# swyoon/Diffusion-by-MaxEntIRL

Hardware: AMD Instinct MI355X
Metric: images/sec (CIFAR-10 DDPM T=10 generation) (higher is better)
Workload: dtype bf16; 1 GPU; CIFAR-10 DDPM U-Net (35.7M params) VARSampler T=10 generation, 256 images/GPU/step, 3x32x32 (BASELINE configs[1]); noise drawn inside the step; global_batch=256, T=10, parallelism=dp1 (independent trajectories, no collective)

## Files before the change

### diffusion-by-maxentirl_amd/csrc/conv_common.h

```cpp
#pragma once
#include "common.h"

struct ConvArgs {
    const bf16* in0;
    const bf16* in1;
    const bf16* w;
    const float* bias;
    const float* addvec;
    const bf16* residual;
    const bf16* mask_src;
    void* out;
    int N, IH, IW, C0, C1, OH, OW, Cout;
    int ksize, stride, pad, ups, act, addvec_ld, in_mode, out_mode;
    int P, pre_act;
    int TWl, THl, SUBS;
    int HH, HWd;
    int PT, CT, CB, KST;
    int tile_px;
    int lds_buf;
    float mask_slope;
    int stagger;
    int RP, SP;
    float* gn_stats;
    bf16* gn_out;
    const float* gn_gamma;
    const float* gn_beta;
    float gn_eps;
    int gn_flags;
    int res_is_mask;
    int xcd_order;
};

__device__ __forceinline__ int dxmi_xcd_logical(int b, int G, int on) {
    if (!on) return b;
    const int x = b & 7, k = b >> 3;
    const int q = G >> 3, r = G & 7;
    return x * q + (x < r ? x : r) + k;
}

__device__ __forceinline__ float dxmi_row16_sum(float t) {
#define DXMI_DPP_ADD(ctrl) t += __builtin_bit_cast(float, __builtin_amdgcn_update_dpp(0, __builtin_bit_cast(int, t), ctrl, 0xf, 0xf, false))
    DXMI_DPP_ADD(0xB1);
    DXMI_DPP_ADD(0x4E);
    DXMI_DPP_ADD(0x141);
    DXMI_DPP_ADD(0x140);
#undef DXMI_DPP_ADD
    return t;
}

__device__ __forceinline__ void dxmi_stats4(const bf16x4& o, float (&st)[4]) {
    const bf16x2 lo = {o[0], o[1]}, hi = {o[2], o[3]};
    const bf16x2 one = {(bf16)1.f, (bf16)1.f};
    st[0] = __builtin_amdgcn_fdot2_f32_bf16(lo, one, st[0], false);
    st[1] = __builtin_amdgcn_fdot2_f32_bf16(lo, lo, st[1], false);
    st[2] = __builtin_amdgcn_fdot2_f32_bf16(hi, one, st[2], false);
    st[3] = __builtin_amdgcn_fdot2_f32_bf16(hi, hi, st[3], false);
}

__device__ __forceinline__ bool conv_block_to_tile(const ConvArgs& p, int bid, int& pt, int& cot) {
    const int xcd = bid & 7;
    const int j = bid >> 3;
    pt = (j / p.CT) * 8 + xcd;
    cot = j % p.CT;
// ... 132 lines not shown
```

### diffusion-by-maxentirl_amd/csrc/conv_head.hip

```cpp
#include "conv_common.h"

namespace {

#define HD_GPTR(p) ((const __attribute__((address_space(1))) void*)(p))
#define HD_LPTR(p) ((__attribute__((address_space(3))) void*)(p))

constexpr int HD_TH = 4;
constexpr int HD_HP = 34, HD_HH = HD_TH + 2, HD_PIX = HD_HP * HD_HH;
constexpr int HD_BLOCKS = (HD_PIX + 3) / 4;

__device__ uint4 hd_zero16 = {0u, 0u, 0u, 0u};

__global__ __launch_bounds__(256, 2) void conv_head_kernel(ConvArgs p) {
    extern __shared__ __attribute__((aligned(1024))) char smem[];
    const int tid = threadIdx.x, lane = tid & 63;
    const int wave = __builtin_amdgcn_readfirstlane(tid >> 6);
    const int txn = p.OW / 32, tyn = p.OH / HD_TH;
    const int tx = blockIdx.x % txn, ty = (blockIdx.x / txn) % tyn, n = blockIdx.x / (txn * tyn);
    const int oy0 = ty * HD_TH, ox0 = tx * 32;

    for (int b = wave; b < HD_BLOCKS; b += 4) {
        const int hp = b * 4 + (lane >> 4);
        const int hy = hp / HD_HP, hx = hp - hy * HD_HP;
        const int iy = oy0 - 1 + hy, ix = ox0 - 1 + hx;
        const int s = (lane & 15) ^ (hp & 15);
        const bool ok = hp < HD_PIX && iy >= 0 && ix >= 0 && iy < p.IH && ix < p.IW;
        const void* g = ok ? (const void*)(p.in0 + (((size_t)n * p.IH + iy) * p.IW + ix) * 128 + s * 8) : (const void*)&hd_zero16;
        __builtin_amdgcn_global_load_lds(HD_GPTR(g), HD_LPTR(smem + b * 1024), 16, 0, 0);
    }
    bf16x8 A[36];
    {
        const int kg = lane >> 4;
        const bf16x8* wf = reinterpret_cast<const bf16x8*>(p.w) + (lane & 15) + 32 * (kg & 1);
#pragma unroll
        for (int t = 0; t < 9; ++t)
#pragma unroll
            for (int c = 0; c < 4; ++c) A[t * 4 + c] = wf[(size_t)((t * p.KST + c * 2 + (kg >> 1)) * p.CB) * 64];
    }
    asm volatile("s_waitcnt vmcnt(0)\n\ts_barrier" ::: "memory");

    constexpr int NBW = HD_TH / 2;
    const int px = lane & 15, kg = lane >> 4;
    f32x4 acc[NBW];
#pragma unroll
    for (int nb = 0; nb < NBW; ++nb)
#pragma unroll
        for (int e = 0; e < 4; ++e) acc[nb][e] = 0.f;
#pragma unroll
    for (int t = 0; t < 9; ++t) {
        const int ky = t / 3, kx = t % 3;
#pragma unroll
        for (int nb = 0; nb < NBW; ++nb) {
            const int hp = (wave * (HD_TH / 4) + (nb >> 1) + ky) * HD_HP + (nb & 1) * 16 + px + kx;
            const char* row = smem + hp * 256;
            const int sw = hp & 15;
#pragma unroll
            for (int c = 0; c < 4; ++c) {
                const bf16x8 b = *reinterpret_cast<const bf16x8*>(row + (((c * 4 + kg) ^ sw) << 4));
                acc[nb] = __builtin_amdgcn_mfma_f32_16x16x32_bf16(A[t * 4 + c], b, acc[nb], 0, 0, 0);
            }
        }
    }
    const float slope = dxmi_act_slope(p.act);
#pragma unroll
    for (int nb = 0; nb < NBW; ++nb) {
        const int oy = oy0 + wave * (HD_TH / 4) + (nb >> 1), ox = ox0 + (nb & 1) * 16 + px;
#pragma unroll
        for (int e = 0; e < 4; ++e) {
            const int co = 4 * kg + e;
            if (co < p.Cout) {
                float v = acc[nb][e] + (p.bias ? p.bias[co] : 0.f);
                v = dxmi_act_lin(v, slope);
                reinterpret_cast<float*>(p.out)[(((size_t)n * p.Cout + co) * p.OH + oy) * p.OW + ox] = v;
            }
        }
    }
}

}

bool conv_head_select(const ConvArgs& a, ConvPlan* p) {
    if (a.in_mode != DXMI_IN_NHWC_BF16 || a.out_mode != DXMI_OUT_NCHW_F32) return false;
    if (a.ksize != 3 || a.stride != 1 || a.pad != 1 || a.ups != 0 || a.mask_src || a.addvec || a.residual || a.act == DXMI_ACT_SILU) return false;
    if (a.C0 != 128 || a.C1 != 0 || a.Cout > 16 || a.OW % 32 != 0 || a.OH % HD_TH != 0) return false;
    p->kind = ConvKernel::head;
    p->grid = a.N * (a.OH / HD_TH) * (a.OW / 32);
    p->lds = (size_t)HD_BLOCKS * 1024;
    p->id = 600000;
    return true;
}

int conv_head_launch(const ConvPlan& p, hipStream_t st) {
    static bool attr_set = false;
    if (!attr_set) {
        (void)hipFuncSetAttribute(reinterpret_cast<const void*>(conv_head_kernel), hipFuncAttributeMaxDynamicSharedMemorySize, 160 * 1024);
        attr_set = true;
    }
    hipLaunchKernelGGL(conv_head_kernel, dim3(p.grid), dim3(256), p.lds, st, p.args);
    DXMI_CHECK_LAUNCH("dxmi_conv2d_fwd(head)");
    return DXMI_OK;
}
```

### diffusion-by-maxentirl_amd/csrc/conv_igemm.hip

```cpp
#include "conv_common.h"

namespace {

template <int MB, int NB, int CK, int PMAX>
__global__ __launch_bounds__(256) void conv_igemm_kernel(ConvArgs p) {
    constexpr int WAVES_PX = 8 / NB;
    constexpr int WAVES_CO = 4 / WAVES_PX;
    constexpr int BN = 32 * MB * WAVES_CO;
    constexpr int ROWB = CK * 2 + 16;
    constexpr int KSTEPS = CK / 16;
    constexpr int PPP = CK / 8;
    extern __shared__ __attribute__((aligned(16))) char smem[];

    const int tid = threadIdx.x;
    const int lane = tid & 63;
    const int wave = __builtin_amdgcn_readfirstlane(tid >> 6);
    const int wco = wave % WAVES_CO;
    const int wpx = wave / WAVES_CO;

    int pt, cot;
    if (!conv_block_to_tile(p, blockIdx.x, pt, cot)) return;

    const bool k27 = p.in_mode == DXMI_IN_NCHW_F32_K27;
    const bool rows = p.in_mode == DXMI_IN_ROWS_F32;
    const int TW = 1 << p.TWl, TH = 1 << p.THl;
    int n0 = 0, oy0 = 0, ox0 = 0;
    if (!rows) {
        const int txn = p.OW >> p.TWl, tyn = p.OH >> p.THl;
        const int tx = pt % txn;
        const int ty = (pt / txn) % tyn;
        n0 = (pt / (txn * tyn)) * p.SUBS;
        oy0 = ty << p.THl;
        ox0 = tx << p.TWl;
// ... 436 lines not shown
    DXMI_CHECK_ARG(!d->addvec || d->addvec_ld == 0 || d->addvec_ld >= d->Cout,
                   "dxmi_conv2d_fwd: addvec_ld %d is neither 0 (one shared row) nor >= Cout %d", d->addvec_ld, d->Cout);
    DXMI_CHECK_ARG((d->OW & (d->OW - 1)) == 0 && (d->OH & (d->OH - 1)) == 0 && d->OW >= 4 && d->OH >= 4,
                   "dxmi_conv2d_fwd: OH/OW must be powers of two >= 4 (got %dx%d)", d->OH, d->OW);
    if (k27) {
        DXMI_CHECK_ARG(d->C0 == 3 && d->C1 == 0 && d->ksize == 3 && d->stride == 1 && d->pad == 1 && !d->upsample &&
                           d->IH == d->OH && d->IW == d->OW,
                       "dxmi_conv2d_fwd: K27 mode needs a 3-channel 3x3/s1/p1 conv");
    } else {
        DXMI_CHECK_ARG(Cin % 32 == 0 && d->C0 % 32 == 0, "dxmi_conv2d_fwd: Cin (%d+%d) must be a multiple of 32", d->C0, d->C1);
        DXMI_CHECK_ARG(d->C1 == 0 || d->in1, "dxmi_conv2d_fwd: C1>0 but in1 is NULL");
        DXMI_CHECK_ARG(d->upsample >= 0 && d->upsample <= 2, "dxmi_conv2d_fwd: upsample must be 0, 1 (nearest) or 2 (zero-stuffed)");
        const int VIH = d->IH << (d->upsample ? 1 : 0), VIW = d->IW << (d->upsample ? 1 : 0);
        DXMI_CHECK_ARG((d->OH - 1) * d->stride - d->pad < VIH && (d->OW - 1) * d->stride - d->pad < VIW && d->pad >= 0 && d->pad < d->ksize,
                       "dxmi_conv2d_fwd: output %dx%d inconsistent with input %dx%d", d->OH, d->OW, VIH, VIW);
    }
    DXMI_CHECK_ARG(d->out_mode != DXMI_OUT_NCHW_F32 || !d->residual, "dxmi_conv2d_fwd: residual unsupported with NCHW output");
    DXMI_CHECK_ARG(!d->residual || d->Cout % 4 == 0, "dxmi_conv2d_fwd: residual needs Cout%%4==0");
    DXMI_CHECK_ARG(!d->mask_src || (d->Cout % 4 == 0 && d->out_mode == DXMI_OUT_NHWC_BF16), "dxmi_conv2d_fwd: mask_src needs NHWC bf16 output, Cout%%4==0");

    ConvArgs a = {};
    a.in0 = (const bf16*)d->in0; a.in1 = (const bf16*)d->in1; a.w = (const bf16*)d->wpacked;
    a.bias = d->bias; a.addvec = d->addvec; a.residual = (const bf16*)d->residual; a.out = d->out;
    a.mask_src = (const bf16*)d->mask_src; a.mask_slope = d->mask_slope; a.gn_stats = d->gn_stats;
    a.gn_out = (bf16*)d->gn_out; a.gn_gamma = d->gn_gamma; a.gn_beta = d->gn_beta; a.gn_eps = d->gn_eps; a.gn_flags = d->gn_flags;
    DXMI_CHECK_ARG(!d->gn_out || (d->gn_gamma && d->gn_beta && d->gn_groups > 0 && d->Cout == 8 * d->gn_groups && d->variant == 0 &&
                                  d->out_mode == DXMI_OUT_NHWC_BF16),
                   "dxmi_conv2d_fwd: gn_out needs gamma / beta, 8 channels per group, the default variant and NHWC bf16 output");
    DXMI_CHECK_ARG(!d->gn_stats || (d->variant == 0 && d->out_mode == DXMI_OUT_NHWC_BF16 && d->Cout % 4 == 0),
                   "dxmi_conv2d_fwd: gn_stats needs the default variant, NHWC bf16 output and Cout%%4==0");
    a.N = d->N; a.IH = d->IH; a.IW = d->IW; a.C0 = d->C0; a.C1 = d->C1; a.OH = d->OH; a.OW = d->OW; a.Cout = d->Cout;
    a.ksize = d->ksize; a.stride = d->stride; a.pad = d->pad; a.ups = d->upsample; a.act = d->act;
    a.addvec_ld = d->addvec_ld; a.in_mode = d->in_mode; a.out_mode = d->out_mode;
    const int TW = d->OW < 32 ? d->OW : 32;
    int TH = 256 / TW; if (TH > d->OH) TH = d->OH;
    a.TWl = ilog2(TW); a.THl = ilog2(TH); a.SUBS = 256 / (TW * TH);
    if (k27) { a.HH = TH; a.HWd = TW; }
    else { a.HH = (TH - 1) * d->stride + d->ksize; a.HWd = (TW - 1) * d->stride + d->ksize; }
    const int ngroups = (d->N + a.SUBS - 1) / a.SUBS;
    a.PT = ngroups * (d->OH / TH) * (d->OW / TW);
    a.CB = (d->Cout + 31) / 32;
    a.KST = k27 ? 2 : Cin / 16;
    conv_select(a, d->variant, p);
    DXMI_CHECK_ARG(!a.gn_out || p->gn_out, "dxmi_conv2d_fwd: the kernel for this shape cannot fuse the GroupNorm of its output "
                                          "(dxmi_conv2d_gn_fuse_supported returns 0 for it)");
    DXMI_CHECK_ARG(!a.gn_stats || p->stats_tile, "dxmi_conv2d_fwd: the kernel for this shape does not emit GroupNorm block statistics "
                                                "(dxmi_conv2d_gn_stats_partials returns 0 for it)");
    DXMI_CHECK_ARG(p->lds <= 160 * 1024, "dxmi_conv2d_fwd: LDS image %zu too large", p->lds);
    return DXMI_OK;
}

extern "C" int dxmi_conv2d_fwd(const dxmi_conv_desc* d, void* stream) {
    ConvPlan p;
    const int rc = conv_plan(d, &p);
    return rc == DXMI_OK ? conv_launch(p, (hipStream_t)stream) : rc;
}

extern "C" int dxmi_conv2d_gn_stats_partials(const dxmi_conv_desc* d) {
    if (!d || d->variant != 0 || d->out_mode != DXMI_OUT_NHWC_BF16) return 0;
    dxmi_conv_desc q = *d;
    q.gn_stats = nullptr;
    ConvPlan p;
    return conv_plan(&q, &p) == DXMI_OK && p.stats_tile ? d->OH * d->OW / p.stats_tile : 0;
}

extern "C" int dxmi_conv2d_gn_fuse_supported(const dxmi_conv_desc* d) {
    if (!d || d->variant != 0 || d->out_mode != DXMI_OUT_NHWC_BF16 || d->gn_groups <= 0 || d->Cout != 8 * d->gn_groups) return 0;
    dxmi_conv_desc q = *d;
    q.gn_stats = nullptr;
    q.gn_out = nullptr;
    ConvPlan p;
    return conv_plan(&q, &p) == DXMI_OK && p.gn_out ? 1 : 0;
}

extern "C" int dxmi_conv2d_kernel_id(const dxmi_conv_desc* d) {
    ConvPlan p;
    const int rc = conv_plan(d, &p);
    return rc == DXMI_OK ? p.id : rc;
}

namespace {
__global__ __launch_bounds__(256) void linear_small_kernel(const float* __restrict__ x, const bf16* __restrict__ w,
                                                          const float* __restrict__ bias, float* __restrict__ out, int P, int K,
                                                          int M, int CB, int pre_act, int post_act, int ksplit) {
    const int lane = threadIdx.x & 63;
    const int wave = __builtin_amdgcn_readfirstlane(threadIdx.x >> 6);
    const int cb = blockIdx.y * 4 + wave;
    if (cb >= CB) return;
// ... 34 lines not shown
        }
    }
    if (!rvalid) return;
#pragma unroll
    for (int g = 0; g < 4; ++g) {
        const int co = cb * 32 + 8 * g + 4 * h;
        if (co + 3 < M) {
            f32x4 o;
#pragma unroll
            for (int e = 0; e < 4; ++e) o[e] = dxmi_act(acc[4 * g + e] + (bias ? bias[co + e] : 0.f), post_act);
            *reinterpret_cast<f32x4*>(out + (size_t)row * M + co) = o;
        } else {
            for (int e = 0; e < 4; ++e)
                if (co + e < M) out[(size_t)row * M + co + e] = dxmi_act(acc[4 * g + e] + (bias ? bias[co + e] : 0.f), post_act);
        }
    }
}
}

extern "C" int dxmi_linear_fwd(const float* x, const void* wpacked, const float* bias, float* out, int32_t P,
                               int32_t K, int32_t M, int32_t pre_act, int32_t post_act, void* stream) {
    DXMI_CHECK_ARG(x && wpacked && out, "dxmi_linear_fwd: null pointer");
    DXMI_CHECK_ARG(P > 0 && M > 0 && K > 0 && K % 32 == 0, "dxmi_linear_fwd: K (%d) must be a positive multiple of 32", K);
    if (P <= 4096 && M % 4 == 0) {
        const int CB = (M + 31) / 32;
        hipLaunchKernelGGL(linear_small_kernel, dim3((P + 31) / 32, (CB + 3) / 4), dim3(256), 0, (hipStream_t)stream, x,
                           (const bf16*)wpacked, bias, out, P, K, M, CB, pre_act, post_act, K / 16);
        DXMI_CHECK_LAUNCH("dxmi_linear_fwd(small)");
        return DXMI_OK;
    }
    ConvArgs a;
    a.in0 = (const bf16*)x; a.in1 = nullptr; a.w = (const bf16*)wpacked; a.bias = bias; a.addvec = nullptr;
    a.residual = nullptr; a.out = out; a.mask_src = nullptr; a.mask_slope = 0.f; a.gn_stats = nullptr; a.gn_out = nullptr;
    a.gn_gamma = a.gn_beta = nullptr; a.gn_eps = 0.f; a.gn_flags = 0; a.res_is_mask = 0;
    a.N = 1; a.IH = 1; a.IW = P; a.C0 = K; a.C1 = 0; a.OH = 1; a.OW = P; a.Cout = M;
    a.ksize = 1; a.stride = 1; a.pad = 0; a.ups = 0; a.act = post_act; a.addvec_ld = 0;
    a.in_mode = DXMI_IN_ROWS_F32; a.out_mode = DXMI_OUT_ROWS_F32; a.P = P; a.pre_act = pre_act;
    a.TWl = 5; a.THl = 3; a.SUBS = 1; a.HH = 8; a.HWd = 32;
    a.PT = (P + 255) / 256; a.CB = (M + 31) / 32; a.KST = K / 16;
    ConvPlan p;
    conv_select(a, 0, &p);
    return conv_launch(p, (hipStream_t)stream);
}

extern "C" int dxmi_linear_splitk_slices(int32_t P, int32_t K, int32_t M) {
    if (P <= 0 || K <= 0 || M <= 0 || K % 32 != 0 || P > 4096 || M % 4 != 0) return 0;
    const long waves = (long)((P + 31) / 32) * ((M + 31) / 32);
    if (K < 4096 || waves >= 1024) return 1;
    int s = (int)(2048 / waves);
    const int smax = K / 16 / 32;
    if (s > smax) s = smax;
    if (s > 64) s = 64;
    return s < 1 ? 1 : s;
}

extern "C" int dxmi_linear_splitk(const float* x, const void* wpacked, float* partials, int32_t P, int32_t K, int32_t M, int32_t pre_act,
                                  void* stream) {
    DXMI_CHECK_ARG(x && wpacked && partials, "dxmi_linear_splitk: null pointer");
    const int S = dxmi_linear_splitk_slices(P, K, M);
    DXMI_CHECK_ARG(S >= 1, "dxmi_linear_splitk: unsupported shape P=%d K=%d M=%d (P <= 4096, M %% 4 == 0, K %% 32 == 0)", P, K, M);
    const int CB = (M + 31) / 32;
    const int ksplit = ((K / 16 + S - 1) / S + 7) / 8 * 8;
    hipLaunchKernelGGL(linear_small_kernel, dim3((P + 31) / 32, (CB + 3) / 4, S), dim3(256), 0, (hipStream_t)stream, x, (const bf16*)wpacked,
                       (const float*)nullptr, partials, P, K, M, CB, pre_act, DXMI_ACT_NONE, ksplit);
    DXMI_CHECK_LAUNCH("dxmi_linear_splitk");
    return DXMI_OK;
}
// ... 1 lines not shown
```

### diffusion-by-maxentirl_amd/dxmi_hip/_lib.py

```python
import ctypes
import os

_HERE = os.path.dirname(os.path.abspath(__file__))
LIB_PATH = os.environ.get("DXMI_LIB") or os.path.join(_HERE, "libdxmi_hip.so")

c_void_p, c_int, c_float, c_int64 = ctypes.c_void_p, ctypes.c_int32, ctypes.c_float, ctypes.c_int64


class ConvDesc(ctypes.Structure):

    _fields_ = [
        ("in0", c_void_p), ("in1", c_void_p), ("wpacked", c_void_p), ("bias", c_void_p),
        ("addvec", c_void_p), ("residual", c_void_p), ("out", c_void_p),
        ("N", c_int), ("IH", c_int), ("IW", c_int), ("C0", c_int), ("C1", c_int),
        ("OH", c_int), ("OW", c_int), ("Cout", c_int),
        ("ksize", c_int), ("stride", c_int), ("pad", c_int), ("upsample", c_int), ("act", c_int),
        ("addvec_ld", c_int), ("in_mode", c_int), ("out_mode", c_int), ("variant", c_int),
        ("mask_src", c_void_p), ("mask_slope", c_float), ("gn_stats", c_void_p),
        ("gn_out", c_void_p), ("gn_gamma", c_void_p), ("gn_beta", c_void_p), ("gn_eps", c_float), ("gn_groups", c_int), ("gn_flags", c_int),
    ]


class PackItem(ctypes.Structure):

    _fields_ = [("w", c_void_p), ("dst", c_void_p), ("Cout", c_int), ("Cin", c_int), ("ksize", c_int), ("transpose_flip", c_int),
                ("k27", c_int)]


SIGNATURES = {
    "dxmi_last_error": (ctypes.c_char_p, []),
    "dxmi_version": (c_int, []),
    "dxmi_device_check": (c_int, []),
    "dxmi_set_tuning": (c_int, [ctypes.c_char_p, c_int]),
    "dxmi_get_tuning": (c_int, [ctypes.c_char_p, ctypes.POINTER(c_int)]),
    "dxmi_conv2d_fwd": (c_int, [ctypes.POINTER(ConvDesc), c_void_p]),
    "dxmi_conv2d_kernel_id": (c_int, [ctypes.POINTER(ConvDesc)]),
    "dxmi_conv2d_gn_stats_partials": (c_int, [ctypes.POINTER(ConvDesc)]),
    "dxmi_conv2d_gn_fuse_supported": (c_int, [ctypes.POINTER(ConvDesc)]),
    "dxmi_conv_ws_last_clock": (c_int, [ctypes.POINTER(ctypes.c_uint64)]),
    "dxmi_gn_block_stats_partials": (c_int, [c_int]),
    "dxmi_gn_block_stats": (c_int, [c_void_p, c_void_p, c_int, c_int, c_int, c_void_p]),
    "dxmi_gn_stats_fold": (c_int, [c_void_p, c_void_p, c_int, c_int, c_int, c_int, c_void_p]),
    "dxmi_groupnorm_apply": (c_int, [c_void_p, c_int, c_void_p, c_int, c_void_p, c_int, c_void_p, c_int, c_void_p, c_void_p, c_void_p, c_int,
                                     c_void_p, c_int, c_int, c_int, c_float, c_int, c_void_p]),
    "dxmi_groupnorm_apply_split": (c_int, [c_void_p, c_int, c_void_p, c_int, c_void_p, c_int, c_void_p, c_int, c_void_p, c_void_p, c_void_p, c_int,
                                           c_void_p, c_void_p, c_int, c_int, c_int, c_float, c_int, c_void_p]),
    "dxmi_groupnorm_silu_shortcut_supported": (c_int, [ctypes.POINTER(ConvDesc), c_int]),
    "dxmi_groupnorm_silu_shortcut": (c_int, [ctypes.POINTER(ConvDesc), c_void_p, c_int, c_void_p, c_int, c_void_p, c_void_p, c_int, c_float,
                                             c_int, c_void_p, c_void_p, c_void_p]),
    "dxmi_gn_blockstats_to_generic": (c_int, [c_void_p, c_int, c_int, c_void_p, c_int, c_int, c_void_p, c_int, c_int, c_int, c_void_p]),
    "dxmi_attention_fwd_lse_supported": (c_int, [c_int, c_int, c_int]),
    "dxmi_attention_fwd_lse": (c_int, [c_void_p, c_void_p, c_void_p, c_int, c_int, c_int, c_int, c_float, c_void_p]),
    "dxmi_attention_bwd_lse": (c_int, [c_void_p, c_void_p, c_void_p, c_void_p, c_void_p, c_void_p, c_int, c_int, c_int, c_int, c_float, c_void_p]),
    "dxmi_gn_ss_grads": (c_int, [c_void_p, c_void_p, c_int, c_void_p, c_void_p, c_void_p, c_void_p, c_void_p, c_int, c_int, c_void_p]),
    "dxmi_fid_stats_workspace_bytes": (c_int64, [c_int64, c_int]),
    "dxmi_fid_stats": (c_int, [c_void_p, c_int64, c_int, c_void_p, c_void_p, c_void_p, c_void_p]),
    "dxmi_knn_radii_workspace_bytes": (c_int64, [c_int64, c_int, c_int, c_int]),
    "dxmi_knn_radii": (c_int, [c_void_p, c_int64, c_int, c_int, c_int, c_void_p, c_void_p, c_void_p]),
    "dxmi_pr_membership_workspace_bytes": (c_int64, [c_int64, c_int64]),
    "dxmi_pr_membership": (c_int, [c_void_p, c_int64, c_void_p, c_void_p, c_int64, c_void_p, c_int, c_void_p, c_void_p, c_void_p, c_void_p]),
    "dxmi_inception_score_workspace_bytes": (c_int64, [c_int64, c_int, c_int]),
    "dxmi_inception_score": (c_int, [c_void_p, c_int64, c_int, c_void_p, c_int, c_int, c_void_p, c_void_p, c_void_p]),
    "dxmi_packed_conv_weight_bytes": (c_int64, [c_int, c_int, c_int, c_int]),
    "dxmi_pack_conv_weights": (c_int, [ctypes.POINTER(PackItem), c_int, c_void_p]),
    "dxmi_pack_conv_weight": (c_int, [c_void_p, c_void_p, c_int, c_int, c_int, c_int, c_int, c_void_p]),
    "dxmi_conv2d_wgrad_workspace_bytes": (c_int64, [c_int] * 6),
    "dxmi_conv2d_wgrad_plan": (c_int, [c_int] * 12 + [c_void_p]),
    "dxmi_conv2d_wgrad": (c_int, [c_void_p, c_int, c_void_p, c_int, c_void_p, c_void_p, c_void_p] + [c_int] * 11 + [c_void_p]),
    "dxmi_conv2d_wgrad_bias": (c_int, [c_void_p, c_int, c_void_p, c_int, c_void_p, c_void_p, c_void_p, c_void_p] + [c_int] * 11 + [c_void_p]),
    "dxmi_groupnorm_silu_bwd": (c_int, [c_void_p, c_int, c_void_p, c_int] + [c_void_p] * 9 + [c_int, c_int, c_int, c_float, c_int, c_void_p]),
    "dxmi_bgemm_bf16": (c_int, [c_void_p, c_void_p, c_void_p, c_int, c_int, c_int, c_int64, c_int64, c_int, c_int, c_int64, c_int64, c_int, c_int, c_int64, c_int64, c_int, c_int, c_float, c_int, c_int, c_void_p]),
# ... 116 lines not shown
```

### diffusion-by-maxentirl_amd/dxmi_hip/ops.py

```python
import ctypes
import os

import torch

from . import _lib
from . import graph as _graph
from ._lib import ConvDesc, check, load

ACT_NONE, ACT_LEAKY02, ACT_RELU, ACT_SILU = 0, 1, 2, 3
IN_NHWC_BF16, IN_NCHW_F32_K27 = 0, 1
OUT_NHWC_BF16, OUT_NCHW_F32 = 0, 1


_RAW_STREAM = getattr(torch._C, "_cuda_getCurrentRawStream", None)
_GET_DEVICE = getattr(torch._C, "_cuda_getDevice", None)


def _stream():
    if _RAW_STREAM is not None and _GET_DEVICE is not None:
        return ctypes.c_void_p(_RAW_STREAM(_GET_DEVICE()))
    return ctypes.c_void_p(torch.cuda.current_stream().cuda_stream)


def _tree_fingerprint(module):
# ... 182 lines not shown

def pack_conv_weight(w, transpose_flip=False, k27=False, out=None):
    _need_cuda(w)
    if w.dim() == 2:
        w = w[:, :, None, None]
    w = w.detach().contiguous().float()
    O, I, k, _ = w.shape
    Cout, Cin = (I, O) if transpose_flip else (O, I)
    lib = load()
    nbytes = lib.dxmi_packed_conv_weight_bytes(Cout, Cin, k, int(k27))
    if out is None:
        out = pack_tensor(nbytes, torch.uint8, w.device)
    assert out.numel() == nbytes
    if _PACK_BATCH is not None:
        _PACK_BATCH.append((w, out, Cout, Cin, k, transpose_flip, k27))
    else:
        check(lib.dxmi_pack_conv_weight(_ptr(w), _ptr(out), Cout, Cin, k, int(transpose_flip), int(k27), _stream()),
              "dxmi_pack_conv_weight")
    return PackedConvWeight(out, Cout, Cin, k, k27, transpose_flip)


class BlockStats:

    __slots__ = ("buf", "P")

    def __init__(self, buf, P):
        self.buf, self.P = buf, P


_STATS_P = {}


def conv2d(x, pw, *, in1=None, bias=None, addvec=None, residual=None, stride=1, pad=None, pad_br=None, upsample=False,
           act=ACT_NONE, out=None, out_nchw_f32=False, variant=0, mask_src=None, mask_slope=0.0, want_stats=False, fuse_gn=None):
    _need_cuda(x, in1, bias, addvec, residual, out)
    k = pw.ksize
    if pad is None:
        pad = k // 2
    d = ConvDesc()
    if pw.k27:
        N, _, IH, IW = x.shape
        C0, C1 = 3, 0
        assert x.dtype == torch.float32 and x.is_contiguous()
    else:
        N, IH, IW, C0 = x.shape
        C1 = in1.shape[3] if in1 is not None else 0
        assert x.dtype == torch.bfloat16 and x.is_contiguous()
        assert in1 is None or (in1.dtype == torch.bfloat16 and in1.is_contiguous() and in1.shape[:3] == x.shape[:3])
        assert C0 + C1 == pw.Cin, f"conv2d: input channels {C0}+{C1} != packed Cin {pw.Cin}"
    VIH, VIW = (IH * 2, IW * 2) if upsample else (IH, IW)
    if pad_br is None:
        pad_br = pad
    OH, OW = (VIH + pad + pad_br - k) // stride + 1, (VIW + pad + pad_br - k) // stride + 1
    Cout = pw.Cout
    if out is None:
        if out_nchw_f32:
            out = torch.empty((N, Cout, OH, OW), dtype=torch.float32, device=x.device)
        else:
            out = torch.empty((N, OH, OW, Cout), dtype=torch.bfloat16, device=x.device)
    d.in0, d.in1, d.wpacked = x.data_ptr(), (in1.data_ptr() if in1 is not None else None), pw.buf.data_ptr()
    d.bias = bias.data_ptr() if bias is not None else None
    if addvec is not None:
        assert addvec.dtype == torch.float32 and addvec.stride(-1) == 1
        d.addvec = addvec.data_ptr()
        d.addvec_ld = addvec.stride(0) if addvec.dim() == 2 else 0
    else:
        d.addvec, d.addvec_ld = None, 0
    if residual is not None:
# ... 4 lines not shown
    d.ksize, d.stride, d.pad, d.upsample, d.act = k, stride, pad, int(upsample), act
    d.in_mode = IN_NCHW_F32_K27 if pw.k27 else IN_NHWC_BF16
    d.out_mode = OUT_NCHW_F32 if out_nchw_f32 else OUT_NHWC_BF16
    d.variant = variant
    if mask_src is not None:
        assert mask_src.dtype == torch.bfloat16 and mask_src.is_contiguous() and tuple(mask_src.shape) == (N, OH, OW, Cout)
    d.mask_src = mask_src.data_ptr() if mask_src is not None else None
    d.mask_slope = float(mask_slope)
    d.gn_stats = None
    stats = None
    if want_stats and not out_nchw_f32 and variant == 0:
        key = (N, IH, IW, C0, C1, OH, OW, Cout, k, stride, pad, int(upsample), act, d.in_mode, residual is not None, mask_src is not None)
        P = _STATS_P.get(key)
        if P is None:
            P = _STATS_P[key] = int(load().dxmi_conv2d_gn_stats_partials(ctypes.byref(d)))
        if P > 0:
            stats = BlockStats(torch.empty((N, P, Cout // 2, 2), dtype=torch.float32, device=x.device), P)
            d.gn_stats = stats.buf.data_ptr()
    d.gn_out, y = None, None
    if fuse_gn is not None:
        assert not want_stats
        gamma, beta, groups, eps, silu, keep_raw = fuse_gn
        d.gn_groups = groups
        d.gn_flags = int(bool(silu)) | (0 if keep_raw else 2)
        key = ("gn", N, IH, IW, C0, C1, OH, OW, Cout, k, stride, pad, int(upsample), act, d.in_mode, d.out_mode, variant,
               residual is not None, mask_src is not None, groups, bool(keep_raw))
        ok = _STATS_P.get(key)
        if ok is None:
            ok = _STATS_P[key] = int(load().dxmi_conv2d_gn_fuse_supported(ctypes.byref(d)))
        if ok:
            assert gamma.dtype == torch.float32 and beta.dtype == torch.float32 and gamma.numel() == Cout and beta.numel() == Cout
            y = torch.empty((N, OH, OW, Cout), dtype=torch.bfloat16, device=x.device)
            d.gn_out, d.gn_gamma, d.gn_beta, d.gn_eps = y.data_ptr(), gamma.data_ptr(), beta.data_ptr(), float(eps)
    if PROFILER is not None:
        PROFILER.launch_conv(d)
    else:
        check(load().dxmi_conv2d_fwd(ctypes.byref(d), _stream()), "dxmi_conv2d_fwd")
    if fuse_gn is not None:
        return (out if (y is None or fuse_gn[5]) else None), y
    if stats is not None and stats.P > MAX_APPLY_PARTIALS:
        stats = fold_stats(stats)
    return (out, stats) if want_stats else out


class OpProfiler:

    def __init__(self):
        self.records = []

    def bracket(self, cls, name, flops, nbytes, fn):
        e0, e1 = torch.cuda.Event(enable_timing=True), torch.cuda.Event(enable_timing=True)
        e0.record()
        out = fn()
        e1.record()
        self.records.append((cls, name, float(flops), float(nbytes), e0, e1))
        return out

    def launch_conv(self, d):
        lib = load()
        kid = lib.dxmi_conv2d_kernel_id(ctypes.byref(d))
        cin = 27 if d.in_mode == IN_NCHW_F32_K27 else (d.C0 + d.C1) * d.ksize * d.ksize
        flops = 2.0 * d.N * d.OH * d.OW * d.Cout * cin
        in_b = d.N * d.IH * d.IW * (d.C0 + d.C1) * (4 if d.in_mode == IN_NCHW_F32_K27 else 2)
        out_b = d.N * d.OH * d.OW * d.Cout * (4 if d.out_mode == OUT_NCHW_F32 else 2)
        res_b = out_b if d.residual else 0
        if d.gn_out:
            res_b += out_b if not (d.gn_flags & 2) else 0
        w_b = d.Cout * cin * 2
        cls = "conv_other" if kid >= 600000 else "conv1x1" if kid >= 500000 else "conv3x3" if kid >= 400000 else "conv_stem" if kid >= 300000 else ("conv1x1" if kid >= 200000 else ("conv3x3" if kid >= 30000 else "conv_other"))
        if kid == 400008 and d.gn_out:
            kid = 400009
        self.bracket(cls, kid, flops, in_b + out_b + res_b + w_b,
                     lambda: check(lib.dxmi_conv2d_fwd(ctypes.byref(d), _stream()), "dxmi_conv2d_fwd"))

    def summary(self):
# ... 1265 lines not shown
```

### diffusion-by-maxentirl_amd/models/DxMI/unet_small.py

```python
import os

import torch
import torch.nn as nn

from dxmi_hip import ops
from dxmi_hip._lib import DxmiError


def Normalize(in_channels):
    return nn.GroupNorm(num_groups=32, num_channels=in_channels, eps=1e-6, affine=True)


def _conv(cin, cout, k, stride=1, padding=0):
    return nn.Conv2d(cin, cout, kernel_size=k, stride=stride, padding=padding)


class Upsample(nn.Module):

    def __init__(self, in_channels, with_conv):
        super().__init__()
        self.with_conv = with_conv
        if with_conv:
            self.conv = _conv(in_channels, in_channels, 3, 1, 1)

# ... 164 lines not shown
                elif isinstance(m, (Upsample, Downsample)):
                    pk[id(m), "conv"] = ops.pack_conv_weight(m.conv.weight)
            pk["conv_in"] = ops.pack_conv_weight(self.conv_in.weight, k27=(self.in_channels == 3))
            pk["conv_out"] = ops.pack_conv_weight(self.conv_out.weight)
        assert dev.type == "cuda"
        self._pack_bufs = pb.buffers
        return pk

    @staticmethod
    def _same_storage(key, old_key):
        return old_key is not None and len(key) == len(old_key) and all(a[0] == b[0] for a, b in zip(key, old_key))

    def packed(self):
        key = self._param_key()
        if self._packed is None or key != self._packed_key:
            reuse = self._pack_bufs if (self._packed is not None and self._same_storage(key, self._packed_key)) else None
            self._packed, self._packed_key = self._pack(reuse=reuse), key
        return self._packed

    def refresh_packs(self):
        self.packed()
        if getattr(self, "_packed_t", None) is not None:
            from .unet_small_train import _pack_t
            _pack_t(self)

    def prepare_capture(self):
        if getattr(self, "_packed_t", None) is not None:
            for k in [k for k in self._packed_t if k not in self._packed_t_planned]:
                del self._packed_t[k]
        self.refresh_packs()

    FUSE_ATTN_PROJ = True
    FUSE_GN_SHORTCUT = os.environ.get("DXMI_GN_SHORTCUT", "1") != "0"
    FUSE_ATTN_BLOCK = True
    FUSE_GN_SMALL = True
    STREAM_GN_MIN_HW = 256

    def _conv_s(self, x, pw, **kw):
        out, st = ops.conv2d(x, pw, want_stats=True, **kw)
        if st is None and out.shape[1] * out.shape[2] >= self.STREAM_GN_MIN_HW:
            st = ops.block_stats(out)
        return out, st

    def _resblock(self, pk, b, x0, x1, tp, s0=None, s1=None, nxt=None):
        stream = x0.shape[1] * x0.shape[2] >= self.STREAM_GN_MIN_HW
        fused = None
        if isinstance(s0, _Normed):
            assert s0.norm is b.norm1 and x1 is None
            a0 = s0.y
        else:
            if self.FUSE_GN_SHORTCUT and stream and b.in_channels != b.out_channels and not b.use_conv_shortcut:
                fused = ops.groupnorm_silu_shortcut(x0, b.norm1.weight, b.norm1.bias, pk[id(b), "short"], in1=x1, bias=b.nin_shortcut.bias,
                                                    eps=1e-6, silu=True, stats=(s0, s1))
            if fused is not None:
                a0, sc = fused
            else:
                a0 = ops.groupnorm_silu(x0, b.norm1.weight, b.norm1.bias, in1=x1, eps=1e-6, silu=True, stats=(s0, s1))
        off = pk[id(b), "toff"]
        a = None
        if not stream and self.FUSE_GN_SMALL:
            h, a = ops.conv2d(a0, pk[id(b), "conv1"], bias=b.conv1.bias, addvec=tp[:, off:off + b.out_channels],
                              fuse_gn=(b.norm2.weight, b.norm2.bias, 32, 1e-6, True, False))
            sh = None
            if a is None and stream:
                sh = ops.block_stats(h)
        else:
# ... 84 lines not shown
                if len(lvl.attn) > 0:
                    h, sh = self._attn(pk, lvl.attn[i_block], h, sh)
                    tr(f"down.{i_level}.attn.{i_block}", h)
                hs.append((h, sh))
            if i_level != self.num_resolutions - 1:
                ds = lvl.downsample
                hs.append(self._conv_s(hs[-1][0], pk[id(ds), "conv"], bias=ds.conv.bias, stride=2, pad=0, pad_br=1))
                tr(f"down.{i_level}.downsample", hs[-1][0])

        h, sh = hs[-1]
        h, sh = self._resblock(pk, self.mid.block_1, h, None, tp, s0=sh, nxt=(self.mid.attn_1.norm, False))
        tr("mid.block_1", h)
        h, sh = self._attn(pk, self.mid.attn_1, h, sh)
        tr("mid.attn_1", h)
        h, sh = self._resblock(pk, self.mid.block_2, h, None, tp, s0=sh)
        tr("mid.block_2", h)

        for i_level in reversed(range(self.num_resolutions)):
            lvl = self.up[i_level]
            for i_block, blk in enumerate(lvl.block):
                skip, sskip = hs.pop()
                if isinstance(sskip, _Normed):
                    sskip = None
                h, sh = self._resblock(pk, blk, h, skip, tp, s0=sh, s1=sskip)
                tr(f"up.{i_level}.block.{i_block}", h)
                if len(lvl.attn) > 0:
                    h, sh = self._attn(pk, lvl.attn[i_block], h, sh)
                    tr(f"up.{i_level}.attn.{i_block}", h)
            if i_level != 0:
                us = lvl.upsample
                h, sh = self._conv_s(h, pk[id(us), "conv"], bias=us.conv.bias, upsample=True)
                tr(f"up.{i_level}.upsample", h)

        a = ops.groupnorm_silu(h, self.norm_out.weight, self.norm_out.bias, eps=1e-6, silu=True, stats=(sh, None))
        return ops.conv2d(a, pk["conv_out"], bias=self.conv_out.bias, out_nchw_f32=True)
```

### include/dxmi_hip.h

```cpp
#ifndef DXMI_HIP_H
#define DXMI_HIP_H

#include <stdint.h>

#ifdef __cplusplus
extern "C" {
#endif

#define DXMI_OK            0
#define DXMI_EINVAL       -1
#define DXMI_ELAUNCH      -2
#define DXMI_ENODEV       -3

#define DXMI_ACT_NONE      0
#define DXMI_ACT_LEAKY02   1
#define DXMI_ACT_RELU      2
#define DXMI_ACT_SILU      3

#define DXMI_IN_NHWC_BF16     0
#define DXMI_IN_NCHW_F32_K27  1
#define DXMI_IN_ROWS_F32      2
#define DXMI_OUT_NHWC_BF16    0
#define DXMI_OUT_NCHW_F32     1
#define DXMI_OUT_ROWS_F32     2
// ... 2 lines not shown
int dxmi_version(void);
int dxmi_device_check(void);
int dxmi_set_tuning(const char* name, int32_t value);
int dxmi_get_tuning(const char* name, int32_t* value);

typedef struct dxmi_conv_desc {
    const void*  in0;
    const void*  in1;
    const void*  wpacked;
    const float* bias;
    const float* addvec;
    const void*  residual;
    void*        out;
    int32_t N, IH, IW, C0, C1;
    int32_t OH, OW, Cout;
    int32_t ksize;
    int32_t stride;
    int32_t pad;
    int32_t upsample;
    int32_t act;
    int32_t addvec_ld;
    int32_t in_mode;
    int32_t out_mode;
    int32_t variant;
    const void*  mask_src;
    float        mask_slope;
    float*       gn_stats;
    void*        gn_out;
    const float* gn_gamma;
    const float* gn_beta;
    float        gn_eps;
    int32_t      gn_groups;
    int32_t      gn_flags;
} dxmi_conv_desc;

int dxmi_conv2d_fwd(const dxmi_conv_desc* d, void* stream);
int dxmi_conv2d_gn_fuse_supported(const dxmi_conv_desc* d);
int dxmi_conv_ws_last_clock(unsigned long long* host_out4);
int dxmi_conv2d_gn_stats_partials(const dxmi_conv_desc* d);
int dxmi_conv2d_kernel_id(const dxmi_conv_desc* d);

int64_t dxmi_packed_conv_weight_bytes(int32_t Cout, int32_t Cin, int32_t ksize, int32_t k27);
int dxmi_pack_conv_weight(const float* w_oihw, void* dst, int32_t Cout, int32_t Cin,
                          int32_t ksize, int32_t transpose_flip, int32_t k27, void* stream);

#define DXMI_PACK_MAX 32
typedef struct dxmi_pack_item {
    const float* w;
    void*        dst;
    int32_t Cout, Cin, ksize, transpose_flip, k27;
} dxmi_pack_item;
int dxmi_pack_conv_weights(const dxmi_pack_item* items, int32_t count, void* stream);

int64_t dxmi_conv2d_wgrad_workspace_bytes(int32_t N, int32_t OH, int32_t OW, int32_t Cin, int32_t Cout,
                                          int32_t ksize);
int dxmi_conv2d_wgrad(const void* x0, int32_t C0, const void* x1, int32_t C1, const void* dy,
                      float* dw_oihw, void* workspace, int32_t N, int32_t IH, int32_t IW, int32_t OH,
                      int32_t OW, int32_t Cout, int32_t ksize, int32_t stride, int32_t pad, int32_t upsample,
                      int32_t accumulate, void* stream);
#define DXMI_WGRAD_1X1_B128      0
#define DXMI_WGRAD_WS3           1
#define DXMI_WGRAD_WS1           2
#define DXMI_WGRAD_REG3_PF       3
#define DXMI_WGRAD_REG3          4
#define DXMI_WGRAD_REG1_PF       5
#define DXMI_WGRAD_REG1          6
#define DXMI_WGRAD_REDUCE_TAPS4  0
#define DXMI_WGRAD_REDUCE_TAPS16 1
#define DXMI_WGRAD_REDUCE_FLAT4  2
#define DXMI_WGRAD_REDUCE_FLAT16 3
// ... 332 lines not shown
```

Baseline: 6746 images/s.

## Fuse final GroupNorm+SiLU into the output head conv's input load

The final norm_out GroupNorm+SiLU is now applied inside the head conv kernel. A small finalize kernel computes per-channel scale/shift tables, which the kernel loads into LDS and uses to normalize the staged input tile in place before the MMA loop. This removes a full read and write of the 128-channel activation and one elementwise kernel launch. In exchange it adds a finalize launch, extra LDS use and an in-kernel normalize pass that may reduce the head kernel's occupancy.

```diff
diff --git a/diffusion-by-maxentirl_amd/csrc/conv_common.h b/diffusion-by-maxentirl_amd/csrc/conv_common.h
--- a/diffusion-by-maxentirl_amd/csrc/conv_common.h
+++ b/diffusion-by-maxentirl_amd/csrc/conv_common.h
@@ -29,6 +29,8 @@
     int gn_flags;
     int res_is_mask;
     int xcd_order;
+    const float* gn_in_ab;
+    int gn_in_silu;
 };
 
 __device__ __forceinline__ int dxmi_xcd_logical(int b, int G, int on) {
diff --git a/diffusion-by-maxentirl_amd/csrc/conv_head.hip b/diffusion-by-maxentirl_amd/csrc/conv_head.hip
--- a/diffusion-by-maxentirl_amd/csrc/conv_head.hip
+++ b/diffusion-by-maxentirl_amd/csrc/conv_head.hip
@@ -1,4 +1,5 @@
 #include "conv_common.h"
+#include "gn_common.h"
 
 namespace {
 
@@ -8,10 +9,15 @@
 constexpr int HD_TH = 4;
 constexpr int HD_HP = 34, HD_HH = HD_TH + 2, HD_PIX = HD_HP * HD_HH;
 constexpr int HD_BLOCKS = (HD_PIX + 3) / 4;
+constexpr int HD_GN_LDS = (HD_BLOCKS + 16) * 1024;
+static_assert(HD_PIX % 4 == 0 && HD_BLOCKS + 16 >= 64, "whole blocks; the GN read of four blocks stays inside the allocation");
+
+typedef int hd_i4 __attribute__((ext_vector_type(4)));
 
 __device__ uint4 hd_zero16 = {0u, 0u, 0u, 0u};
 
-__global__ __launch_bounds__(256, 2) void conv_head_kernel(ConvArgs p) {
+template <bool GN>
+__device__ __forceinline__ void conv_head_tile(const ConvArgs& p) {
     extern __shared__ __attribute__((aligned(1024))) char smem[];
     const int tid = threadIdx.x, lane = tid & 63;
     const int wave = __builtin_amdgcn_readfirstlane(tid >> 6);
@@ -28,6 +34,14 @@
         const void* g = ok ? (const void*)(p.in0 + (((size_t)n * p.IH + iy) * p.IW + ix) * 128 + s * 8) : (const void*)&hd_zero16;
         __builtin_amdgcn_global_load_lds(HD_GPTR(g), HD_LPTR(smem + b * 1024), 16, 0, 0);
     }
+    if constexpr (GN) {
+        const int s = (lane & 15) ^ ((4 * wave + (lane >> 4)) & 15);
+        const float* q = p.gn_in_ab + ((size_t)n * 128 + s * 8) * 2;
+#pragma unroll
+        for (int i = 0; i < 4; ++i)
+            __builtin_amdgcn_global_load_lds(HD_GPTR(q + 4 * i), HD_LPTR(smem + (HD_BLOCKS + wave * 4 + i) * 1024), 16, 0, 0);
+        asm volatile("" ::: "memory");
+    }
     bf16x8 A[36];
     {
         const int kg = lane >> 4;
@@ -37,7 +51,36 @@
 #pragma unroll
             for (int c = 0; c < 4; ++c) A[t * 4 + c] = wf[(size_t)((t * p.KST + c * 2 + (kg >> 1)) * p.CB) * 64];
     }
-    asm volatile("s_waitcnt vmcnt(0)\n\ts_barrier" ::: "memory");
+    if constexpr (GN) {
+        asm volatile("s_waitcnt vmcnt(36)" ::: "memory");
+        const unsigned lbase = (unsigned)(__UINTPTR_TYPE__)HD_LPTR(smem) + lane * 16;
+        f32x4 t0, t1, t2, t3;
+        asm volatile("ds_read_b128 %0, %4\n\tds_read_b128 %1, %4 offset:1024\n\tds_read_b128 %2, %4 offset:2048\n\t"
+                     "ds_read_b128 %3, %4 offset:3072\n\ts_waitcnt lgkmcnt(0)"
+                     : "=&v"(t0), "=&v"(t1), "=&v"(t2), "=&v"(t3) : "v"(lbase + (HD_BLOCKS + wave * 4) * 1024) : "memory");
+        const float ga[8] = {t0[0], t0[2], t1[0], t1[2], t2[0], t2[2], t3[0], t3[2]};
+        const float gb[8] = {t0[1], t0[3], t1[1], t1[3], t2[1], t2[3], t3[1], t3[3]};
+        for (int b0 = wave; b0 < HD_BLOCKS; b0 += 16) {
+            hd_i4 v[4];
+            asm volatile("ds_read_b128 %0, %4\n\tds_read_b128 %1, %4 offset:4096\n\tds_read_b128 %2, %4 offset:8192\n\t"
+                         "ds_read_b128 %3, %4 offset:12288\n\ts_waitcnt lgkmcnt(0)"
+                         : "=&v"(v[0]), "=&v"(v[1]), "=&v"(v[2]), "=&v"(v[3]) : "v"(lbase + b0 * 1024) : "memory");
+#pragma unroll
+            for (int j = 0; j < 4; ++j) {
+                const int b = b0 + 4 * j;
+                const int hp = b * 4 + (lane >> 4);
+                const int hy = hp / HD_HP, hx = hp - hy * HD_HP;
+                const int iy = oy0 - 1 + hy, ix = ox0 - 1 + hx;
+                if (b < HD_BLOCKS && iy >= 0 && ix >= 0 && iy < p.IH && ix < p.IW) {
+                    const hd_i4 o = __builtin_bit_cast(hd_i4, gn_norm8(__builtin_bit_cast(bf16x8, v[j]), ga, gb, p.gn_in_silu));
+                    asm volatile("ds_write_b128 %0, %1" ::"v"(lbase + b * 1024), "v"(o) : "memory");
+                }
+            }
+        }
+        asm volatile("s_waitcnt vmcnt(0) lgkmcnt(0)\n\ts_barrier" ::: "memory");
+    } else {
+        asm volatile("s_waitcnt vmcnt(0)\n\ts_barrier" ::: "memory");
+    }
 
     constexpr int NBW = HD_TH / 2;
     const int px = lane & 15, kg = lane >> 4;
@@ -77,6 +120,9 @@
     }
 }
 
+__global__ __launch_bounds__(256, 2) void conv_head_kernel(ConvArgs p) { conv_head_tile<false>(p); }
+__global__ __launch_bounds__(256, 2) void conv_head_gn_kernel(ConvArgs p) { conv_head_tile<true>(p); }
+
 }
 
 bool conv_head_select(const ConvArgs& a, ConvPlan* p) {
@@ -85,7 +131,7 @@
     if (a.C0 != 128 || a.C1 != 0 || a.Cout > 16 || a.OW % 32 != 0 || a.OH % HD_TH != 0) return false;
     p->kind = ConvKernel::head;
     p->grid = a.N * (a.OH / HD_TH) * (a.OW / 32);
-    p->lds = (size_t)HD_BLOCKS * 1024;
+    p->lds = a.gn_in_ab ? (size_t)HD_GN_LDS : (size_t)HD_BLOCKS * 1024;
     p->id = 600000;
     return true;
 }
@@ -94,9 +140,11 @@
     static bool attr_set = false;
     if (!attr_set) {
         (void)hipFuncSetAttribute(reinterpret_cast<const void*>(conv_head_kernel), hipFuncAttributeMaxDynamicSharedMemorySize, 160 * 1024);
+        (void)hipFuncSetAttribute(reinterpret_cast<const void*>(conv_head_gn_kernel), hipFuncAttributeMaxDynamicSharedMemorySize, 160 * 1024);
         attr_set = true;
     }
-    hipLaunchKernelGGL(conv_head_kernel, dim3(p.grid), dim3(256), p.lds, st, p.args);
+    if (p.args.gn_in_ab) hipLaunchKernelGGL(conv_head_gn_kernel, dim3(p.grid), dim3(256), p.lds, st, p.args);
+    else hipLaunchKernelGGL(conv_head_kernel, dim3(p.grid), dim3(256), p.lds, st, p.args);
     DXMI_CHECK_LAUNCH("dxmi_conv2d_fwd(head)");
     return DXMI_OK;
 }
diff --git a/diffusion-by-maxentirl_amd/csrc/conv_igemm.hip b/diffusion-by-maxentirl_amd/csrc/conv_igemm.hip
--- a/diffusion-by-maxentirl_amd/csrc/conv_igemm.hip
+++ b/diffusion-by-maxentirl_amd/csrc/conv_igemm.hip
@@ -1,4 +1,5 @@
 #include "conv_common.h"
+#include "gn_common.h"
 
 namespace {
 
@@ -501,6 +502,15 @@
     a.N = d->N; a.IH = d->IH; a.IW = d->IW; a.C0 = d->C0; a.C1 = d->C1; a.OH = d->OH; a.OW = d->OW; a.Cout = d->Cout;
     a.ksize = d->ksize; a.stride = d->stride; a.pad = d->pad; a.ups = d->upsample; a.act = d->act;
     a.addvec_ld = d->addvec_ld; a.in_mode = d->in_mode; a.out_mode = d->out_mode;
+    if (d->gn_in_stats) {
+        DXMI_CHECK_ARG(d->gn_in_gamma && d->gn_in_beta && d->gn_in_ab && d->gn_in_P > 0,
+                       "dxmi_conv2d_fwd: gn_in_stats needs gamma / beta, the table workspace gn_in_ab and gn_in_P > 0");
+        DXMI_CHECK_ARG(d->gn_in_groups > 0 && d->gn_in_groups <= 32 && d->C1 == 0 && d->C0 % d->gn_in_groups == 0 &&
+                           (d->C0 / d->gn_in_groups) % 2 == 0 && !k27 && !d->upsample && d->variant == 0,
+                       "dxmi_conv2d_fwd: gn_in needs one NHWC bf16 source, 1..32 groups of an even channel count (C0 %d, groups %d) and "
+                       "the default variant", d->C0, d->gn_in_groups);
+        a.gn_in_ab = d->gn_in_ab; a.gn_in_silu = d->gn_in_flags & 1;
+    }
     const int TW = d->OW < 32 ? d->OW : 32;
     int TH = 256 / TW; if (TH > d->OH) TH = d->OH;
     a.TWl = ilog2(TW); a.THl = ilog2(TH); a.SUBS = 256 / (TW * TH);
@@ -515,14 +525,29 @@
                                           "(dxmi_conv2d_gn_fuse_supported returns 0 for it)");
     DXMI_CHECK_ARG(!a.gn_stats || p->stats_tile, "dxmi_conv2d_fwd: the kernel for this shape does not emit GroupNorm block statistics "
                                                 "(dxmi_conv2d_gn_stats_partials returns 0 for it)");
+    DXMI_CHECK_ARG(!a.gn_in_ab || p->kind == ConvKernel::head, "dxmi_conv2d_fwd: the kernel for this shape cannot apply a GroupNorm to its "
+                                                              "input on load (dxmi_conv2d_gn_in_supported returns 0 for it)");
     DXMI_CHECK_ARG(p->lds <= 160 * 1024, "dxmi_conv2d_fwd: LDS image %zu too large", p->lds);
     return DXMI_OK;
 }
 
 extern "C" int dxmi_conv2d_fwd(const dxmi_conv_desc* d, void* stream) {
     ConvPlan p;
-    const int rc = conv_plan(d, &p);
+    int rc = conv_plan(d, &p);
+    if (rc == DXMI_OK && d->gn_in_stats)
+        rc = gn_finalize_launch(d->gn_in_stats, d->gn_in_P, d->C0, nullptr, 0, 0, d->gn_in_gamma, d->gn_in_beta, d->gn_in_ab, d->N,
+                                d->IH * d->IW, d->gn_in_groups, d->gn_in_eps, (hipStream_t)stream);
     return rc == DXMI_OK ? conv_launch(p, (hipStream_t)stream) : rc;
+}
+
+extern "C" int dxmi_conv2d_gn_in_supported(const dxmi_conv_desc* d) {
+    if (!d || d->variant != 0 || d->C1 != 0 || d->gn_in_groups <= 0 || d->gn_in_groups > 32 || d->C0 % d->gn_in_groups != 0 ||
+        (d->C0 / d->gn_in_groups) % 2 != 0)
+        return 0;
+    dxmi_conv_desc q = *d;
+    q.gn_in_stats = nullptr;
+    ConvPlan p;
+    return conv_plan(&q, &p) == DXMI_OK && p.kind == ConvKernel::head ? 1 : 0;
 }
 
 extern "C" int dxmi_conv2d_gn_stats_partials(const dxmi_conv_desc* d) {
@@ -623,7 +648,7 @@
     ConvArgs a;
     a.in0 = (const bf16*)x; a.in1 = nullptr; a.w = (const bf16*)wpacked; a.bias = bias; a.addvec = nullptr;
     a.residual = nullptr; a.out = out; a.mask_src = nullptr; a.mask_slope = 0.f; a.gn_stats = nullptr; a.gn_out = nullptr;
-    a.gn_gamma = a.gn_beta = nullptr; a.gn_eps = 0.f; a.gn_flags = 0; a.res_is_mask = 0;
+    a.gn_gamma = a.gn_beta = nullptr; a.gn_eps = 0.f; a.gn_flags = 0; a.res_is_mask = 0; a.gn_in_ab = nullptr; a.gn_in_silu = 0;
     a.N = 1; a.IH = 1; a.IW = P; a.C0 = K; a.C1 = 0; a.OH = 1; a.OW = P; a.Cout = M;
     a.ksize = 1; a.stride = 1; a.pad = 0; a.ups = 0; a.act = post_act; a.addvec_ld = 0;
     a.in_mode = DXMI_IN_ROWS_F32; a.out_mode = DXMI_OUT_ROWS_F32; a.P = P; a.pre_act = pre_act;
diff --git a/diffusion-by-maxentirl_amd/dxmi_hip/_lib.py b/diffusion-by-maxentirl_amd/dxmi_hip/_lib.py
--- a/diffusion-by-maxentirl_amd/dxmi_hip/_lib.py
+++ b/diffusion-by-maxentirl_amd/dxmi_hip/_lib.py
@@ -18,6 +18,8 @@
         ("addvec_ld", c_int), ("in_mode", c_int), ("out_mode", c_int), ("variant", c_int),
         ("mask_src", c_void_p), ("mask_slope", c_float), ("gn_stats", c_void_p),
         ("gn_out", c_void_p), ("gn_gamma", c_void_p), ("gn_beta", c_void_p), ("gn_eps", c_float), ("gn_groups", c_int), ("gn_flags", c_int),
+        ("gn_in_stats", c_void_p), ("gn_in_gamma", c_void_p), ("gn_in_beta", c_void_p), ("gn_in_ab", c_void_p), ("gn_in_eps", c_float),
+        ("gn_in_P", c_int), ("gn_in_groups", c_int), ("gn_in_flags", c_int),
     ]
 
 
@@ -37,6 +39,7 @@
     "dxmi_conv2d_kernel_id": (c_int, [ctypes.POINTER(ConvDesc)]),
     "dxmi_conv2d_gn_stats_partials": (c_int, [ctypes.POINTER(ConvDesc)]),
     "dxmi_conv2d_gn_fuse_supported": (c_int, [ctypes.POINTER(ConvDesc)]),
+    "dxmi_conv2d_gn_in_supported": (c_int, [ctypes.POINTER(ConvDesc)]),
     "dxmi_conv_ws_last_clock": (c_int, [ctypes.POINTER(ctypes.c_uint64)]),
     "dxmi_gn_block_stats_partials": (c_int, [c_int]),
     "dxmi_gn_block_stats": (c_int, [c_void_p, c_void_p, c_int, c_int, c_int, c_void_p]),
diff --git a/diffusion-by-maxentirl_amd/dxmi_hip/ops.py b/diffusion-by-maxentirl_amd/dxmi_hip/ops.py
--- a/diffusion-by-maxentirl_amd/dxmi_hip/ops.py
+++ b/diffusion-by-maxentirl_amd/dxmi_hip/ops.py
@@ -238,8 +238,14 @@
 
 
 def conv2d(x, pw, *, in1=None, bias=None, addvec=None, residual=None, stride=1, pad=None, pad_br=None, upsample=False,
-           act=ACT_NONE, out=None, out_nchw_f32=False, variant=0, mask_src=None, mask_slope=0.0, want_stats=False, fuse_gn=None):
+           act=ACT_NONE, out=None, out_nchw_f32=False, variant=0, mask_src=None, mask_slope=0.0, want_stats=False, fuse_gn=None,
+           gn_in=None):
     _need_cuda(x, in1, bias, addvec, residual, out)
+    if gn_in is not None:
+        gamma, beta, groups, eps, silu, st = gn_in
+        if not _gn_in_supported(x, pw, in1, pad, pad_br, stride, upsample, act, out_nchw_f32, variant, groups, st):
+            x = groupnorm_silu(x, gamma, beta, groups=groups, eps=eps, silu=silu, stats=(st, None))
+            gn_in = None
     k = pw.ksize
     if pad is None:
         pad = k // 2
@@ -310,6 +316,13 @@
             assert gamma.dtype == torch.float32 and beta.dtype == torch.float32 and gamma.numel() == Cout and beta.numel() == Cout
             y = torch.empty((N, OH, OW, Cout), dtype=torch.bfloat16, device=x.device)
             d.gn_out, d.gn_gamma, d.gn_beta, d.gn_eps = y.data_ptr(), gamma.data_ptr(), beta.data_ptr(), float(eps)
+    if gn_in is not None:
+        gamma, beta, groups, eps, silu, st = gn_in
+        assert gamma.dtype == torch.float32 and beta.dtype == torch.float32 and gamma.numel() == C0 and beta.numel() == C0
+        assert tuple(st.buf.shape) == (N, st.P, C0 // 2, 2)
+        ab = torch.empty((N, C0, 2), dtype=torch.float32, device=x.device)
+        d.gn_in_stats, d.gn_in_gamma, d.gn_in_beta, d.gn_in_ab = st.buf.data_ptr(), gamma.data_ptr(), beta.data_ptr(), ab.data_ptr()
+        d.gn_in_eps, d.gn_in_P, d.gn_in_groups, d.gn_in_flags = float(eps), st.P, groups, int(bool(silu))
     if PROFILER is not None:
         PROFILER.launch_conv(d)
     else:
@@ -319,6 +332,27 @@
     if stats is not None and stats.P > MAX_APPLY_PARTIALS:
         stats = fold_stats(stats)
     return (out, stats) if want_stats else out
+
+
+def _gn_in_supported(x, pw, in1, pad, pad_br, stride, upsample, act, out_nchw_f32, variant, groups, st):
+    if not isinstance(st, BlockStats) or pw.k27 or in1 is not None or upsample or x.dim() != 4:
+        return False
+    N, IH, IW, C0 = x.shape
+    k = pw.ksize
+    pad = k // 2 if pad is None else pad
+    pad_br = pad if pad_br is None else pad_br
+    key = ("gn_in", N, IH, IW, C0, pw.Cout, k, stride, pad, pad_br, act, bool(out_nchw_f32), variant, groups)
+    ok = _STATS_P.get(key)
+    if ok is None:
+        d = ConvDesc()
+        d.in0 = d.wpacked = d.out = 16
+        d.N, d.IH, d.IW, d.C0, d.C1, d.Cout = N, IH, IW, C0, 0, pw.Cout
+        d.OH, d.OW = (IH + pad + pad_br - k) // stride + 1, (IW + pad + pad_br - k) // stride + 1
+        d.ksize, d.stride, d.pad, d.upsample, d.act = k, stride, pad, 0, act
+        d.in_mode, d.out_mode = IN_NHWC_BF16, (OUT_NCHW_F32 if out_nchw_f32 else OUT_NHWC_BF16)
+        d.variant, d.gn_in_groups = variant, groups
+        ok = _STATS_P[key] = int(load().dxmi_conv2d_gn_in_supported(ctypes.byref(d)))
+    return bool(ok)
 
 
 class OpProfiler:
diff --git a/diffusion-by-maxentirl_amd/models/DxMI/unet_small.py b/diffusion-by-maxentirl_amd/models/DxMI/unet_small.py
--- a/diffusion-by-maxentirl_amd/models/DxMI/unet_small.py
+++ b/diffusion-by-maxentirl_amd/models/DxMI/unet_small.py
@@ -220,6 +220,7 @@
 
     FUSE_ATTN_PROJ = True
     FUSE_GN_SHORTCUT = os.environ.get("DXMI_GN_SHORTCUT", "1") != "0"
+    FUSE_GN_HEAD = os.environ.get("DXMI_GN_HEAD", "1") != "0"
     FUSE_ATTN_BLOCK = True
     FUSE_GN_SMALL = True
     STREAM_GN_MIN_HW = 256
@@ -370,5 +371,8 @@
                 h, sh = self._conv_s(h, pk[id(us), "conv"], bias=us.conv.bias, upsample=True)
                 tr(f"up.{i_level}.upsample", h)
 
+        if self.FUSE_GN_HEAD and isinstance(sh, ops.BlockStats):
+            return ops.conv2d(h, pk["conv_out"], bias=self.conv_out.bias, out_nchw_f32=True,
+                              gn_in=(self.norm_out.weight, self.norm_out.bias, 32, 1e-6, True, sh))
         a = ops.groupnorm_silu(h, self.norm_out.weight, self.norm_out.bias, eps=1e-6, silu=True, stats=(sh, None))
         return ops.conv2d(a, pk["conv_out"], bias=self.conv_out.bias, out_nchw_f32=True)
diff --git a/include/dxmi_hip.h b/include/dxmi_hip.h
--- a/include/dxmi_hip.h
+++ b/include/dxmi_hip.h
@@ -58,10 +58,19 @@
     float        gn_eps;
     int32_t      gn_groups;
     int32_t      gn_flags;
+    const float* gn_in_stats;
+    const float* gn_in_gamma;
+    const float* gn_in_beta;
+    float*       gn_in_ab;
+    float        gn_in_eps;
+    int32_t      gn_in_P;
+    int32_t      gn_in_groups;
+    int32_t      gn_in_flags;
 } dxmi_conv_desc;
 
 int dxmi_conv2d_fwd(const dxmi_conv_desc* d, void* stream);
 int dxmi_conv2d_gn_fuse_supported(const dxmi_conv_desc* d);
+int dxmi_conv2d_gn_in_supported(const dxmi_conv_desc* d);
 int dxmi_conv_ws_last_clock(unsigned long long* host_out4);
 int dxmi_conv2d_gn_stats_partials(const dxmi_conv_desc* d);
 int dxmi_conv2d_kernel_id(const dxmi_conv_desc* d);
```

Result: no change. 6798 images/s (median of 6 runs) (+0.8%).
